# AlanPearl/multigrad

Hardware: AMD Instinct MI355X
Metric: Adam steps/sec (whole node), 1e7-param summed-loss model (higher is better)
Workload: dtype fp32; 1 GPU; global_batch=134217728, seq_len=10, parallelism=dp1, params=10000000, halos_global=134217728, optimizer=Adam (fused HIP kernel), full trajectory, graph=False, graph_steps=0, pipelined=True, placement=hashed, grad_collective=none (1 rank), sumstat_allreduce=none (1 rank), chunks=1, layout=lanes/global, bounds=none

## Files before the change

multigrad_amd/csrc/smf.hip:

```cpp
#include "common.h"
#include "twoshot.h"
#include "xgmi.h"
#include "tail_table.h"

#include <torch/extension.h>
#include <ATen/hip/HIPContext.h>
#include <cmath>
#include <vector>

namespace mg {

constexpr int kMaxBins = 32;
constexpr int kXcds = 8;
constexpr int kThreads = 256;
static_assert(kThreads == kTsThreads, "fused-exchange kernels must launch kTsThreads threads");
constexpr int kItems = 8;
constexpr int kTileHalos = kThreads * kItems;
constexpr int kTilePops = 2048;
constexpr float kLn10 = 2.302585092994046f;
constexpr float kLog2_10 = 3.321928094887362f;

struct SmfBins {
  float edge[kMaxBins + 1];
  float scale[kMaxBins];
// ... 646 lines not shown
    G[i] = G[i] + g;
    W[i] = (-g) * n + W[i];
  }
}

template <int NB, bool LOGSIG, bool REL, bool RESID, int REPL = 0>
__device__ __forceinline__ void lane_halo_ep(float x0, float x1, float ninv, float mua,
                                             const SmfBins& b,
                                             v2f (&acc)[EdgePairs<NB>::NV], int (&cnt)[NB + 1],
                                             v2f (&G)[EdgePairs<NB>::NV],
                                             v2f (&W)[EdgePairs<NB>::NV],
                                             const float4* tb = nullptr) {
  using E = EdgePairs<NB>;
  auto eval = [&](v2f n, int i, int& ca, int& cb) {
    if constexpr (REPL > 0)
      ep_eval_tab<NB, RESID, REPL>(n, tb, acc, G, W, i, ca, cb);
    else
      ep_eval<NB, REL, RESID>(n, acc, G, W, i, ca, cb);
  };
  const float mu0 = fmaf(x0, -ninv, mua);
  const float mu1 = fmaf(x1, -ninv, mua);
#pragma unroll
  for (int h = 0; h < 2; ++h) {
    const float mu = h ? mu1 : mu0;
#pragma unroll
    for (int i = 0; i < E::NP; ++i) {
      v2f e2;
      e2.x = b.edge[2 * i];
      e2.y = b.edge[2 * i + 1];
      const v2f n = e2 * ninv + mu;
      eval(n, i, cnt[2 * i], cnt[2 * i + 1]);
    }
  }
  if constexpr (E::NX) {
    v2f m2;
    m2.x = mu0;
    m2.y = mu1;
    const v2f n = (v2f)(b.edge[E::NE - 1] * ninv) + m2;
    int c2 = 0;
    eval(n, E::NP, cnt[E::NE - 1], c2);
    cnt[E::NE - 1] += c2;
  }
}

constexpr float kEmHMax = 0.5f;
constexpr float kInvSqrt2Pi = 0.39894228040143268f;

struct EmLane {
  float inv;
  float dw4;
  float a1, a3, a5;
};

__device__ __forceinline__ EmLane em_lane(float inv, float delta) {
  constexpr float ik = 1.0f / kWScale;
  EmLane L;
  L.inv = inv;
  const float dw = delta * inv;
  L.dw4 = -4.0f * dw;
  const float h = dw * ik;
  const float h2 = h * h, h4 = h2 * h2, h6 = h4 * h2;
  L.a1 = (h2 * (1.0f / 12.0f) + h4 * (3.0f / 720.0f) + h6 * (15.0f / 30240.0f)) * ik;
  L.a3 = -(h4 * (1.0f / 720.0f) + h6 * (10.0f / 30240.0f)) * (ik * ik * ik);
  L.a5 = h6 * (1.0f / 30240.0f) * (ik * ik * ik * ik * ik);
  return L;
}

constexpr float kEmH2 = 0.35f;

__device__ __forceinline__ EmLane em_lane2(float inv, float delta) {
  constexpr float ik = 1.0f / kWScale;
  EmLane L;
  L.inv = inv;
  const float dw = delta * inv;
  L.dw4 = -4.0f * dw;
  const float h = dw * ik;
  const float h2 = h * h, h4 = h2 * h2;
  L.a1 = (h2 * (1.0f / 12.0f) + h4 * (3.0f / 720.0f)) * ik;
  L.a3 = -(h4 * (1.0f / 720.0f)) * (ik * ik * ik);
  L.a5 = 0.0f;
  return L;
}

template <int NB, bool RESID, bool A7 = false, bool A5 = true>
__device__ __forceinline__ void em_halo(float nm, float inv, float dw4, float a1, float a3,
                                        float a5, const SmfBins& b,
                                        v2f (&F)[EdgePairs<NB>::NV], v2f (&Wa)[EdgePairs<NB>::NV],
                                        v2f (&E)[EdgePairs<NB>::NV], float a7 = 0.0f) {
  using EP = EdgePairs<NB>;
  constexpr int M = EP::NP / 2;
  nm = __builtin_amdgcn_fmed3f(nm, -1e6f, 1e6f);
  const float dw2 = -0.5f * dw4;
  v2f wm;
  {
    v2f e2;
    e2.x = b.edge[2 * M];
    e2.y = b.edge[2 * M + 1];
    wm = e2 * inv + nm;
  }
  auto wpair = [&](int i) { return wm + (float)(i - M) * dw2; };
  auto accum = [&](int i, v2f p, v2f w) {
    const v2f pw = p * w;
    F[i] = F[i] + p;
    if constexpr (RESID) Wa[i] = Wa[i] + pw;
    const v2f w2 = w * w;
    v2f t;
    if constexpr (A7) {
      t = w2 * a7 + a5;
      t = t * w2 + a3;
      t = t * w2 + a1;
    } else if constexpr (A5) {
      t = w2 * a5 + a3;
      t = t * w2 + a1;
    } else {
      t = w2 * a3 + a1;
    }
    E[i] = pw * t + E[i];
  };
  const v2f ws = wpair(M);
  const v2f q = -ws * ws;
  v2f p0;
  p0.x = fast_exp2(q.x);
  p0.y = fast_exp2(q.y);
  const float R = fast_exp2(__builtin_amdgcn_fmed3f(dw4 * ws.y, -126.0f, 126.0f));
  accum(M, p0, ws);
  v2f p = p0;
#pragma unroll
  for (int i = M + 1; i < EP::NP; ++i) {
    p = p * R;
    accum(i, p, wpair(i));
  }
  if constexpr (EP::NX) {
    const float pz = p.x * R;
    const float wz = fmaf((float)(EP::NP - M), dw2, wm.x);
    const float pw = pz * wz;
    F[EP::NP].x += pz;
    if constexpr (RESID) Wa[EP::NP].x += pw;
    const float w2 = wz * wz;
    const float t = A7 ? fmaf(fmaf(fmaf(w2, a7, a5), w2, a3), w2, a1)
                       : (A5 ? fmaf(fmaf(w2, a5, a3), w2, a1) : fmaf(w2, a3, a1));
    E[EP::NP].x = fmaf(pw, t, E[EP::NP].x);
  }
  if constexpr (M > 0) {
    const float Ri = fast_rcp(R);
    p = p0;
#pragma unroll
    for (int i = M - 1; i >= 0; --i) {
      p = p * Ri;
      accum(i, p, wpair(i));
    }
  }
}

template <int NB, bool RESID, bool A5 = true>
__device__ __forceinline__ void lane_halo_em(float x, const EmLane& L, float nma,
                                             const SmfBins& b, v2f (&F)[EdgePairs<NB>::NV],
                                             v2f (&Wa)[EdgePairs<NB>::NV],
                                             v2f (&E)[EdgePairs<NB>::NV]) {
  em_halo<NB, RESID, false, A5>(fmaf(x, -L.inv, nma), L.inv, L.dw4, L.a1, L.a3, L.a5, b, F, Wa, E);
  __builtin_amdgcn_sched_barrier(0);
}

template <int NB, bool RESID>
__device__ __forceinline__ void lane_halo_exact1(float x, float ninv, float mua, const SmfBins& b,
                                                 v2f (&acc)[EdgePairs<NB>::NV], int (&cnt)[NB + 1],
                                                 v2f (&G)[EdgePairs<NB>::NV],
                                                 v2f (&W)[EdgePairs<NB>::NV]) {
  const float mu = fmaf(x, -ninv, mua);
#pragma unroll
  for (int e = 0; e <= NB; ++e) {
    const float n = fmaf(b.edge[e], ninv, mu);
    float p, g;
    normal_tail_parts_w<false>(n, p, g);
    const float v = p * __builtin_copysignf(g, n);
    cnt[e] += __builtin_popcountll(__builtin_amdgcn_ballot_w64(n < 0.0f));
    const int i = e >> 1;
    if (e & 1) {
      acc[i].y += v;
      if constexpr (RESID) {
        G[i].y += g;
        W[i].y = fmaf(-g, n, W[i].y);
      }
    } else {
      acc[i].x += v;
      if constexpr (RESID) {
        G[i].x += g;
        W[i].x = fmaf(-g, n, W[i].x);
      }
    }
  }
  __builtin_amdgcn_sched_barrier(0);
}

template <int NB, class LaneT>
__device__ __forceinline__ void em_group_end(const LaneT& L, v2f (&F)[EdgePairs<NB>::NV],
                                             v2f (&Wa)[EdgePairs<NB>::NV],
                                             v2f (&E)[EdgePairs<NB>::NV],
                                             v2f (&accp)[EdgePairs<NB>::NV]) {
  using EP = EdgePairs<NB>;
  constexpr int M = EP::NP / 2;
  const float l4 = 0.25f * L.dw4 * L.dw4;
#pragma unroll
  for (int i = 0; i < EP::NV; ++i) {
    const int j = i - M;
    v2f Q;
    Q.x = (j * (j - 1) == 0) ? 1.0f : fast_exp2(-l4 * (float)(j * (j - 1)));
    Q.y = (i == EP::NP) ? Q.x : ((j * j == 0) ? 1.0f : fast_exp2(-l4 * (float)(j * j)));
    F[i] = F[i] * Q;
    Wa[i] = Wa[i] * Q;
    E[i] = E[i] * Q;
  }
  const float hh = (-0.125f / kWScale) * L.dw4;
  float T = 0.0f, fprev = 0.0f;
#pragma unroll
  for (int e = 0; e <= NB; ++e) {
    const int i = e >> 1;
    float fe, ee;
    if (i < EP::NP) {
      fe = (e & 1) ? F[i].y : F[i].x;
      ee = (e & 1) ? E[i].y : E[i].x;
    } else {
      fe = F[i].x + F[i].y;
      ee = E[i].x + E[i].y;
    }
    if (e > 0) T = fmaf(hh, fprev + fe, T);
    fprev = fe;
    const float C = kInvSqrt2Pi * (T + ee);
    if (i < EP::NP) {
      if (e & 1) accp[i].y += C;
      else accp[i].x += C;
    } else {
      accp[i].x += C;
    }
  }
}


template <int NB>
struct VjpPairs {
  v2f h[EdgePairs<NB>::NV];
  v2f d[EdgePairs<NB>::NV];
};

template <int NB>
__device__ __forceinline__ void halo_vjp_rec(float nm, float inv, float dw, const VjpPairs<NB>& W,
                                             const SmfBins& b, float& A, float& D, float& wc) {
  using EP = EdgePairs<NB>;
  constexpr int M = EP::NP / 2;
  v2f e2;
  e2.x = b.edge[2 * M];
  e2.y = b.edge[2 * M + 1];
  const v2f ws = e2 * inv + nm;
  const v2f q = -ws * ws;
  v2f p0;
  p0.x = fast_exp2(q.x);
  p0.y = fast_exp2(q.y);
  const float dw4 = -4.0f * dw;
  const float C2 = fast_exp2(dw4 * dw);
  const float C4 = C2 * C2;
  v2f Af = W.h[M] * p0, Df = W.d[M] * p0;
  v2f R;
  R.x = fast_exp2(__builtin_amdgcn_fmed3f(dw4 * ws.y, -126.0f, 126.0f));
  R.y = R.x * C2;
  v2f p = p0;
#pragma unroll
  for (int i = M + 1; i < EP::NP; ++i) {
    p = p * R;
    Af = W.h[i] * p + Af;
    Df = W.d[i] * p + Df;
    R = R * C4;
  }
  if constexpr (EP::NX) {
    const float f = p.x * R.x;
    Af.x = fmaf(W.h[EP::NP].x, f, Af.x);
    Df.x = fmaf(W.d[EP::NP].x, f, Df.x);
  }
  if constexpr (M > 0) {
    v2f Rb;
    Rb.y = fast_exp2(__builtin_amdgcn_fmed3f(-dw4 * ws.x, -126.0f, 126.0f));
    Rb.x = Rb.y * C2;
    p = p0;
#pragma unroll
    for (int i = M - 1; i >= 0; --i) {
      p = p * Rb;
      Af = W.h[i] * p + Af;
      Df = W.d[i] * p + Df;
      Rb = Rb * C4;
    }
  }
  A = Af.x + Af.y;
  D = Df.x + Df.y;
  wc = ws.x;
}

template <int NB, bool LOGSIG, int XS = 0>
#ifndef MG_VJP_REC_MINWAVES
#define MG_VJP_REC_MINWAVES 8
#endif
__global__ __launch_bounds__(kThreads, XS == 2 ? 6 : MG_VJP_REC_MINWAVES) void smf_vjp_tiles_rec_kernel(
    const float* __restrict__ x, const int32_t* __restrict__ pop,
    const float2* __restrict__ theta, const Tile* __restrict__ tiles,
    const float* __restrict__ hvec, SmfBins bins, float2* __restrict__ grad,
    float2* __restrict__ partials, TwoShotPack xs = TwoShotPack{}) {
  __shared__ __attribute__((aligned(16))) char smem[kTileHalos * (sizeof(float2) + sizeof(int16_t))];
  int tb = blockIdx.x;
  if constexpr (XS > 0) {
// ... 22 lines not shown
    block_sum_n<2>(v, reinterpret_cast<float*>(smem));
    if (tid == 0) partials[t.slot] = make_float2(v[0], v[1]);
    return;
  }
  const int n = (int)(t.h1 - t.h0);
  const int npops = t.p1 - t.p0;
  float2* __restrict__ gout = grad + t.p0;
  if (n <= 0) {
    for (int k = tid; k < npops; k += kThreads) gout[k] = make_float2(0.f, 0.f);
    return;
  }
  VjpPairs<NB> W;
#pragma unroll
  for (int i = 0; i < EP::NV; ++i) {
    const int e0 = 2 * i, e1 = 2 * i + 1;
    W.h[i].x = hvec[e0];
    W.h[i].y = e1 <= NB ? hvec[e1] : 0.0f;
    W.d[i].x = (float)(e0 - 2 * M) * W.h[i].x;
    W.d[i].y = (float)(e1 - 2 * M) * W.h[i].y;
  }
  float2* s_g = reinterpret_cast<float2*>(smem);
  int16_t* s_lp = reinterpret_cast<int16_t*>(smem + kTileHalos * sizeof(float2));
  float2* res = s_g;
  float2* s_head = reinterpret_cast<float2*>(s_lp);
  int* s_pass = reinterpret_cast<int*>(s_head + kThreads);
  static_assert(kThreads * (sizeof(float2) + sizeof(int)) <= kTileHalos * sizeof(int16_t),
                "head partials alias the id array");
  static_assert(kTileHalos == kTilePops, "result array aliases the contribution array");
  auto swz = [](int i) { return i ^ (((i >> 5) & 3) << 1); };
  {
    float xs[kItems];
    int ps[kItems];
    float2 ths[kItems];
    const float* __restrict__ xt = x + t.h0;
    const int32_t* __restrict__ pt = pop + t.h0;
#pragma unroll
    for (int r = 0; r < kItems; ++r) {
      const int i = min(r * kThreads + tid, n - 1);
      xs[r] = xt[i];
      ps[r] = pt[i];
    }
#pragma unroll
    for (int r = 0; r < kItems; ++r) ths[r] = theta[ps[r]];
    bool ok = true;
#pragma unroll
    for (int r = 0; r < kItems; ++r) ok = ok && bins.delta * inv_sigma<LOGSIG>(ths[r].y) <= 1.0f;
    constexpr float kInvW = 1.0f / kWScale;
    if (__builtin_amdgcn_ballot_w64(!ok) == 0) {
#pragma unroll
      for (int r = 0; r < kItems; ++r) {
        const float is = inv_sigma<LOGSIG>(ths[r].y);
        const float inv = is * kWScale;
        const float dw = bins.delta * inv;
        float A, D, wc;
        halo_vjp_rec<NB>(-(xs[r] + ths[r].x) * inv, inv, dw, W, bins, A, D, wc);
        const float B = fmaf(wc, A, dw * D);
        const int li = r * kThreads + tid;
        s_g[swz(li)] = make_float2(-is * A, LOGSIG ? -(kLn10 * kInvW) * B : -(is * kInvW) * B);
        s_lp[li] = (int16_t)(ps[r] - t.p0);
      }
    } else {
      float h[NB + 1];
#pragma unroll
      for (int e = 0; e <= NB; ++e) h[e] = hvec[e];
#pragma unroll
      for (int r = 0; r < kItems; ++r) {
        const float is = inv_sigma<LOGSIG>(ths[r].y);
        float A = 0.f, B = 0.f;
        halo_vjp<NB, LOGSIG>(xs[r], ths[r], is * kWScale, h, bins, A, B);
        const int li = r * kThreads + tid;
        s_g[swz(li)] = make_float2(-is * A, LOGSIG ? -(kLn10 * kInvW) * B : -(is * kInvW) * B);
        s_lp[li] = (int16_t)(ps[r] - t.p0);
      }
    }
  }
  __syncthreads();
  const int base = tid * kItems;
  const int cnt = max(0, min(kItems, n - base));
  float2 g[kItems];
  int lp[kItems];
  {
    const float4* sg4 = reinterpret_cast<const float4*>(s_g);
    const int sw = (tid >> 2) & 3;
#pragma unroll
    for (int k = 0; k < kItems / 2; ++k) {
      const float4 v = sg4[4 * tid + (k ^ sw)];
      g[2 * k] = make_float2(v.x, v.y);
      g[2 * k + 1] = make_float2(v.z, v.w);
    }
    const uint4 l4 = reinterpret_cast<const uint4*>(s_lp)[tid];
    const unsigned lw[4] = {l4.x, l4.y, l4.z, l4.w};
#pragma unroll
    for (int k = 0; k < 4; ++k) {
      lp[2 * k] = (int)(lw[k] & 0xFFFFu);
      lp[2 * k + 1] = (int)(lw[k] >> 16);
    }
  }
#pragma unroll
  for (int j = 1; j < kItems; ++j) {
    const bool in = j < cnt;
    lp[j] = in ? lp[j] : lp[j - 1];
    g[j].x = in ? g[j].x : 0.0f;
    g[j].y = in ? g[j].y : 0.0f;
  }
  const int prevlp = (cnt > 0 && base > 0) ? (int)s_lp[base - 1] : -1;
  const int nextlp = base + kItems < n ? (int)s_lp[base + kItems] : npops;
  __syncthreads();
  for (int k = tid; k < npops; k += kThreads) res[k] = make_float2(0.f, 0.f);
  __syncthreads();
  int c = lp[0];
  float2 cur = g[0];
  const bool headcont = cnt > 0 && c == prevlp;
  bool inhead = true;
  float2 hsum = make_float2(0.f, 0.f);
  if (cnt > 0) {
#pragma unroll
    for (int j = 1; j < kItems; ++j) {
      const bool brk = lp[j] != c;
      const bool hb = brk && inhead && headcont;
      if (brk && !hb) res[c] = cur;
      hsum.x = hb ? cur.x : hsum.x;
      hsum.y = hb ? cur.y : hsum.y;
      inhead = inhead && !brk;
      cur.x = brk ? g[j].x : cur.x + g[j].x;
      cur.y = brk ? g[j].y : cur.y + g[j].y;
      c = lp[j];
    }
  }
  const bool contonly = cnt > 0 && inhead && headcont;
  if (contonly) hsum = cur;
  s_head[tid] = hsum;
  s_pass[tid] = contonly && nextlp == c;
  __syncthreads();
  if (cnt > 0 && !contonly) {
    if (nextlp == c) {
      for (int k = tid + 1; k < kThreads; ++k) {
        const float2 hp = s_head[k];
        cur.x += hp.x;
        cur.y += hp.y;
        if (!s_pass[k]) break;
      }
    }
    res[c] = cur;
  }
  __syncthreads();
  for (int k = tid; k < npops; k += kThreads) gout[k] = res[k];
}

constexpr int kLanesMainMode = 3;

#ifndef MG_EM2
#define MG_EM2 1
#endif

#ifndef MG_LANES_MINWAVES
#define MG_LANES_MINWAVES 4
#endif
#ifndef MG_LANES_UNROLL
#define MG_LANES_UNROLL 2
#endif
constexpr int kLanesUnroll = MG_LANES_UNROLL;

__device__ __forceinline__ __amdgpu_buffer_rsrc_t buf_rsrc(const void* p) {
  return __builtin_amdgcn_make_buffer_rsrc(const_cast<void*>(p), (short)0, 0x7fffffff, 0x00020000);
}
__device__ __forceinline__ float buf_load_f32(__amdgpu_buffer_rsrc_t r, int voff, int soff) {
  return __builtin_bit_cast(float, __builtin_amdgcn_raw_buffer_load_b32(r, voff, soff, 0));
}
__device__ __forceinline__ int buf_load_i32(__amdgpu_buffer_rsrc_t r, int voff, int soff) {
  return (int)__builtin_amdgcn_raw_buffer_load_b32(r, voff, soff, 0);
}
__device__ __forceinline__ void buf_store_f32(__amdgpu_buffer_rsrc_t r, int voff, int soff, float v) {
  __builtin_amdgcn_raw_buffer_store_b32(__builtin_bit_cast(unsigned, v), r, voff, soff, 0);
}

struct LaneSrc {
  __amdgpu_buffer_rsrc_t r;
  int voff;
};
__device__ __forceinline__ float lane_load(const LaneSrc& xp, int j, int len) {
  return j < len ? buf_load_f32(xp.r, xp.voff, j * kWave * 4) : kLaneSentinel;
}
__device__ __forceinline__ float lane_use(float v, int j, int len) {
  return v;
}

__device__ __forceinline__ void resid_store(float* p, float v) {
  *p = v;
}

#ifdef MG_FWD_TRACE
constexpr int kTraceWaves = 16384;
__device__ unsigned long long g_fwd_trace[3 * kTraceWaves];
#endif

__device__ __forceinline__ void vmem_wait_all() { __builtin_amdgcn_s_waitcnt(0x0F70); }

template <int I>
__device__ __forceinline__ void lds_stage_chunk(const float* src, float* dst, int lane) {
  constexpr int base = (I / 4) * 1024;
  __builtin_amdgcn_global_load_lds(src + base + lane * 4, dst + base, 16, (I % 4) * 1024, 0);
}
template <int R>
__device__ __forceinline__ void lds_stage_row(const float* src, float* dst, int lane) {
  constexpr int base = (R * kWave / 1024) * 1024;
  __builtin_amdgcn_global_load_lds(src + base + lane, dst + base, 4, (R * kWave - base) * 4, 0);
}
template <int NR, int... I, int... R>
__device__ __forceinline__ void lds_stage_seq(const float* src, float* dst, int lane,
                                              std::integer_sequence<int, I...>,
                                              std::integer_sequence<int, R...>) {
  (lds_stage_chunk<I>(src, dst, lane), ...);
  (lds_stage_row<(NR / 4) * 4 + R>(src, dst, lane), ...);
}
template <int NR>
__device__ __forceinline__ void lds_stage_block(const float* src, float* dst, int lane) {
  lds_stage_seq<NR>(src, dst, lane, std::make_integer_sequence<int, NR / 4>{},
                    std::make_integer_sequence<int, NR % 4>{});
}

template <int NB>
struct LaneGroupSums {
  v2f acc[EdgePairs<NB>::NV];
  int cnt[NB + 1];
};

template <int NB>
__device__ __attribute__((noinline)) LaneGroupSums<NB> lanes_group_exact(
    const float* __restrict__ xg, int len, float x0, float x1, float ninv, float mua, float e0,
    float delta, float* __restrict__ rg) {
  using EP = EdgePairs<NB>;
  const int lane = threadIdx.x & (kWave - 1);
  SmfBins b;
#pragma unroll
  for (int e = 0; e <= NB; ++e) b.edge[e] = fmaf((float)e, delta, e0);
  LaneGroupSums<NB> o;
  v2f G[EP::NV], W[EP::NV];
#pragma unroll
  for (int i = 0; i < EP::NV; ++i) {
    o.acc[i] = (v2f)(0.0f);
    G[i] = (v2f)(0.0f);
    W[i] = (v2f)(0.0f);
  }
#pragma unroll
  for (int e = 0; e <= NB; ++e) o.cnt[e] = 0;
  const __amdgpu_buffer_rsrc_t xr = buf_rsrc(xg);
  const int voff = lane * 4;
  for (int j = 0; j < len; j += 2) {
    const float c0 = x0;
    const float c1 = j + 1 < len ? x1 : kLaneSentinel;
    x0 = buf_load_f32(xr, voff, (j + 2) * kWave * 4);
    x1 = buf_load_f32(xr, voff, (j + 3) * kWave * 4);
    lane_halo_ep<NB, true, false, true>(c0, c1, ninv, mua, b, o.acc, o.cnt, G, W);
  }
  float Gs[NB + 1], Ws[NB + 1];
#pragma unroll
  for (int i = 0; i < EP::NP; ++i) {
    Gs[2 * i] = G[i].x;
    Gs[2 * i + 1] = G[i].y;
    Ws[2 * i] = W[i].x;
    Ws[2 * i + 1] = W[i].y;
  }
  if constexpr (EP::NX) {
    Gs[NB] = G[EP::NP].x + G[EP::NP].y;
    Ws[NB] = W[EP::NP].x + W[EP::NP].y;
  }
  const __amdgpu_buffer_rsrc_t rr = buf_rsrc(rg);
#pragma unroll
  for (int e = 0; e <= NB; ++e) {
    buf_store_f32(rr, voff, e * kWave * 4, Gs[e]);
    buf_store_f32(rr, voff, (NB + 1 + e) * kWave * 4, Ws[e]);
  }
  return o;
}

template <int NB, bool LOGSIG, bool REL, bool RESID, bool UPD = false, int LMODE = 0,
          bool BND = false>
__global__ __launch_bounds__(kThreads, MG_LANES_MINWAVES) void smf_fwd_lanes_kernel(
    const float* __restrict__ xi, const int32_t* __restrict__ slot_pop,
    const int64_t* __restrict__ group_base, const int32_t* __restrict__ group_len,
    const int32_t* __restrict__ fwd_order, const float2* __restrict__ theta, int64_t g0,
    int64_t g1, SmfBins bins, float* __restrict__ slab, float* __restrict__ resid,
    const int32_t* __restrict__ wave_start, int* __restrict__ queues, int nq,
    LanesUpdate upd = LanesUpdate{}) {
  static_assert(!UPD || RESID, "the pipelined update reads the residuals it overwrites");
  static_assert(!BND || UPD, "bounds belong to the pipelined update");
  static_assert(LMODE == 0 || LMODE == 3 || LMODE == 4, "lanes mode");
  static_assert(LMODE != 3 || (RESID && !REL), "CALL: EM residual forwards");
  constexpr bool kEmOn = LMODE != 4;
  constexpr int kRepl = (!REL && !kEmOn && !RESID) ? (UPD ? 8 : 16) : 0;
  constexpr bool kEm = kEmOn && !REL;
  const float4* tb = nullptr;
  if constexpr (kRepl > 0) {
    __shared__ float4 tab[kTailTabN * (kRepl > 0 ? kRepl : 1)];
    tail_tab_fill<kRepl>(tab);
    __syncthreads();
    tb = tail_tab_lane<kRepl>(tab);
  }
  float acc[NB + 1];
  int cnt[NB + 1];
#pragma unroll
  for (int k = 0; k <= NB; ++k) {
    acc[k] = 0.0f;
    cnt[k] = 0;
  }
  using EP = EdgePairs<NB>;
  static_assert(kLanesUnroll % 2 == 0, "edge-pair path takes halos two at a time");
  v2f accp[EP::NV];
#pragma unroll
  for (int k = 0; k < EP::NV; ++k) accp[k] = (v2f)(0.0f);
  const int lane = threadIdx.x & (kWave - 1);
  const int wid = __builtin_amdgcn_readfirstlane(threadIdx.x >> 6);
  const int64_t nwaves = (int64_t)gridDim.x * (kThreads / kWave);
  const int64_t w_id = (int64_t)blockIdx.x * (kThreads / kWave) + wid;
#ifdef MG_FWD_TRACE
  const unsigned long long t_start = __builtin_amdgcn_s_memrealtime();
  int n_groups_done = 0;
#endif
  const bool dyn = queues != nullptr;
  const int qid = dyn ? (int)(blockIdx.x % nq) : 0;
  const int n_items = (int)(g1 - g0);
  const int n_q = dyn && qid < n_items ? (n_items - qid + nq - 1) / nq : 0;
  const int waves_q = dyn ? (kThreads / kWave) * (int)((gridDim.x - qid + nq - 1) / nq) : 0;
  auto draw = [&]() -> int64_t {
    int t = 0;
    if (lane == 0) {
      t = atomicAdd(queues + qid, 1);
      if (t == n_q + waves_q - 1)
        __hip_atomic_store(queues + qid, 0, __ATOMIC_RELAXED, __HIP_MEMORY_SCOPE_AGENT);
    }
    t = __builtin_amdgcn_readfirstlane(t);
    return t < n_q ? g0 + qid + (int64_t)t * nq : g1;
  };
  int64_t k = dyn ? draw() : wave_start ? (int64_t)wave_start[w_id] : g0 + w_id;
  const int64_t kstride = wave_start ? 1 : nwaves;
  if (wave_start && !dyn) g1 = wave_start[w_id + 1];
  int64_t k_next = g1;
  int64_t g = 0;
  float2 th = make_float2(0.f, 0.f);
  const int lane4 = lane * 4;
  LaneSrc xp{buf_rsrc(xi), lane4};
  auto slot_of = [&](int64_t kk) {
    return buf_load_i32(buf_rsrc(slot_pop + (int64_t)fwd_order[kk] * kWave), lane4, 0);
  };
  int len = 0;
  int c_next = 0;
  int c_cur = -1;
  float xn[kLanesUnroll];
  float ubc1 = 1.0f, ubc2 = 1.0f;
  float* utrow = nullptr;
  if constexpr (UPD) {
    const int st = upd.host_step >= 0
                       ? upd.host_step
                       : __hip_atomic_load(upd.step, __ATOMIC_RELAXED, __HIP_MEMORY_SCOPE_AGENT);
    ubc1 = 1.0f / (1.0f - powf(upd.b1, (float)(st + 1)));
    ubc2 = 1.0f / (1.0f - powf(upd.b2, (float)(st + 1)));
    if (upd.traj) utrow = upd.traj + (int64_t)(st + 1) * upd.traj_stride;
  }
  constexpr int kUR = UPD ? 2 * (NB + 1) + 4 + (BND ? 6 : 0) : 1;
  float* ubuf = nullptr;
  const float* uh = nullptr;
  if constexpr (UPD) {
    __shared__ __attribute__((aligned(16))) float ub[(kThreads / kWave) * kUR * kWave];
    __shared__ float hs[NB + 1];
    if (threadIdx.x <= NB) hs[threadIdx.x] = upd.h[threadIdx.x];
    __syncthreads();
    ubuf = ub + wid * (kUR * kWave);
    uh = hs;
  }
  auto stage_update = [&](int64_t gg, int c) {
    if constexpr (UPD) {
      constexpr int NR = 2 * (NB + 1);
      lds_stage_block<NR>(resid + gg * (NR * kWave), ubuf, lane);
      const int64_t j = c < 0 ? 0 : c - upd.unit_offset;
      const float* mp = reinterpret_cast<const float*>(upd.m + j);
      const float* vp = reinterpret_cast<const float*>(upd.v + j);
      __builtin_amdgcn_global_load_lds(mp, ubuf + NR * kWave, 4, 0, 0);
      __builtin_amdgcn_global_load_lds(mp + 1, ubuf + (NR + 1) * kWave, 4, 0, 0);
      __builtin_amdgcn_global_load_lds(vp, ubuf + (NR + 2) * kWave, 4, 0, 0);
      __builtin_amdgcn_global_load_lds(vp + 1, ubuf + (NR + 3) * kWave, 4, 0, 0);
      if constexpr (BND) {
        const float* up = reinterpret_cast<const float*>(upd.u + j);
        const float* lp = reinterpret_cast<const float*>(upd.lo + j);
        const float* hp = reinterpret_cast<const float*>(upd.hi + j);
        __builtin_amdgcn_global_load_lds(up, ubuf + (NR + 4) * kWave, 4, 0, 0);
        __builtin_amdgcn_global_load_lds(up + 1, ubuf + (NR + 5) * kWave, 4, 0, 0);
        __builtin_amdgcn_global_load_lds(lp, ubuf + (NR + 6) * kWave, 4, 0, 0);
        __builtin_amdgcn_global_load_lds(lp + 1, ubuf + (NR + 7) * kWave, 4, 0, 0);
        __builtin_amdgcn_global_load_lds(hp, ubuf + (NR + 8) * kWave, 4, 0, 0);
        __builtin_amdgcn_global_load_lds(hp + 1, ubuf + (NR + 9) * kWave, 4, 0, 0);
      }
    }
  };
  auto apply_update = [&]() {
    if constexpr (UPD) {
      constexpr int NR = 2 * (NB + 1);
      float A = 0.0f, B = 0.0f;
#pragma unroll
      for (int e = 0; e <= NB; ++e) {
        A = fmaf(uh[e], ubuf[e * kWave + lane], A);
        B = fmaf(uh[e], ubuf[(NB + 1 + e) * kWave + lane], B);
      }
      if (c_cur >= 0) {
        const float2 gr = pop_grad<LOGSIG>(th, A, B);
        const int64_t j = c_cur - upd.unit_offset;
        float2 mm = make_float2(ubuf[NR * kWave + lane], ubuf[(NR + 1) * kWave + lane]);
        float2 vv = make_float2(ubuf[(NR + 2) * kWave + lane], ubuf[(NR + 3) * kWave + lane]);
        if constexpr (BND) {
          float2 uu = make_float2(ubuf[(NR + 4) * kWave + lane], ubuf[(NR + 5) * kWave + lane]);
          const float2 lo = make_float2(ubuf[(NR + 6) * kWave + lane], ubuf[(NR + 7) * kWave + lane]);
          const float2 hi = make_float2(ubuf[(NR + 8) * kWave + lane], ubuf[(NR + 9) * kWave + lane]);
          const int8_t kx = bound_kind(lo.x, hi.x), ky = bound_kind(lo.y, hi.y);
          const float gx = gr.x * dpdu_fast(upd.legacy ? th.x : uu.x, lo.x, hi.x, kx);
          const float gy = gr.y * dpdu_fast(upd.legacy ? th.y : uu.y, lo.y, hi.y, ky);
          mm.x = (1.0f - upd.b1) * gx + upd.b1 * mm.x;
          mm.y = (1.0f - upd.b1) * gy + upd.b1 * mm.y;
          vv.x = (1.0f - upd.b2) * (gx * gx) + upd.b2 * vv.x;
          vv.y = (1.0f - upd.b2) * (gy * gy) + upd.b2 * vv.y;
          uu.x -= upd.lr * (mm.x * ubc1) * __builtin_amdgcn_rcpf(__builtin_amdgcn_sqrtf(vv.x * ubc2) + upd.eps);
          uu.y -= upd.lr * (mm.y * ubc1) * __builtin_amdgcn_rcpf(__builtin_amdgcn_sqrtf(vv.y * ubc2) + upd.eps);
          th.x = inv_transform_fast(uu.x, lo.x, hi.x, kx);
          th.y = inv_transform_fast(uu.y, lo.y, hi.y, ky);
          upd.u[j] = uu;
        } else {
          mm.x = (1.0f - upd.b1) * gr.x + upd.b1 * mm.x;
          mm.y = (1.0f - upd.b1) * gr.y + upd.b1 * mm.y;
          vv.x = (1.0f - upd.b2) * (gr.x * gr.x) + upd.b2 * vv.x;
          vv.y = (1.0f - upd.b2) * (gr.y * gr.y) + upd.b2 * vv.y;
          th.x -= upd.lr * (mm.x * ubc1) * __builtin_amdgcn_rcpf(__builtin_amdgcn_sqrtf(vv.x * ubc2) + upd.eps);
          th.y -= upd.lr * (mm.y * ubc1) * __builtin_amdgcn_rcpf(__builtin_amdgcn_sqrtf(vv.y * ubc2) + upd.eps);
        }
        upd.m[j] = mm;
        upd.v[j] = vv;
        upd.theta_w[c_cur] = th;
        if (utrow) reinterpret_cast<float2*>(utrow)[j] = th;
      }
    }
  };
  auto fetch_next_slot = [&]() {
    if (k_next < g1) c_next = slot_of(k_next);
  };
  auto load_group = [&](int64_t kk, int c, bool fetch_next = true) {
    g = fwd_order[kk];
    c_cur = c;
    stage_update(g, c);
    th = theta[c < 0 ? 0 : c];
    xp.r = buf_rsrc(xi + group_base[g]);
    len = group_len[g];
#pragma unroll
    for (int u = 0; u < kLanesUnroll; ++u) xn[u] = lane_load(xp, u, len);
    k_next = dyn ? draw() : kk + kstride;
    if (fetch_next) fetch_next_slot();
  };
  if (k < g1) {
    load_group(k, slot_of(k), !UPD);
    if constexpr (UPD) {
      vmem_wait_all();
      apply_update();
      fetch_next_slot();
    }
  }
  const int64_t k_first = k;
  while (k < g1) {
    if (!dyn && wave_start) {
      const int64_t tot = g1 - k_first;
      const int lvl = (int)((4 * (g1 - k) - 1) / tot);
      if (lvl >= 3) __builtin_amdgcn_s_setprio(3);
      else if (lvl == 2) __builtin_amdgcn_s_setprio(2);
      else if (lvl == 1) __builtin_amdgcn_s_setprio(1);
      else __builtin_amdgcn_s_setprio(0);
    }
    const int64_t gc = g;
    const float ninv = -inv_sigma<LOGSIG>(th.y) * kWScale;
    const float mua = -th.x * ninv;
    v2f Gp[EP::NV], Wp[EP::NV];
#pragma unroll
    for (int e = 0; e < EP::NV; ++e) {
      Gp[e] = (v2f)(0.0f);
      Wp[e] = (v2f)(0.0f);
    }
    bool em = false, em2 = false;
    if constexpr (kEm) {
      const float inv = -ninv;
      const float h = bins.delta * inv * (1.0f / kWScale);
      const bool bad = c_cur >= 0 && !(h <= kEmHMax);
      em = bins.delta > 0.0f && __builtin_amdgcn_ballot_w64(bad) == 0;
#if MG_EM2
      em2 = em && __builtin_amdgcn_ballot_w64(c_cur >= 0 && !(h <= kEmH2)) == 0;
#endif
    }
    if constexpr (kEm) if (em) {
      const EmLane eml = em2 ? em_lane2(-ninv, bins.delta) : em_lane(-ninv, bins.delta);
      v2f Ep[EP::NV];
#pragma unroll
      for (int e = 0; e < EP::NV; ++e) Ep[e] = (v2f)(0.0f);
      auto em_loop = [&](auto a5c) {
        for (int j = 0; j < len; j += kLanesUnroll) {
          float xc[kLanesUnroll];
#pragma unroll
          for (int u = 0; u < kLanesUnroll; ++u) {
            xc[u] = lane_use(xn[u], j + u, len);
            xn[u] = lane_load(xp, j + kLanesUnroll + u, len);
          }
#pragma unroll
          for (int u = 0; u < kLanesUnroll; ++u)
            lane_halo_em<NB, RESID, decltype(a5c)::value>(xc[u], eml, -mua, bins, Gp, Wp, Ep);
        }
      };
      if (em2) em_loop(std::false_type{});
      else em_loop(std::true_type{});
      em_group_end<NB>(eml, Gp, Wp, Ep, accp);
    }
    if constexpr (LMODE == 3) {
      if (!em) {
        const LaneGroupSums<NB> o = lanes_group_exact<NB>(
            xi + group_base[gc], len, lane_use(xn[0], 0, len), lane_use(xn[1], 1, len), ninv,
            mua, bins.edge[0], bins.delta,
            resid + gc * (2 * (NB + 1) * kWave));
#pragma unroll
        for (int i = 0; i < EP::NV; ++i) accp[i] = accp[i] + o.acc[i];
#pragma unroll
        for (int e = 0; e <= NB; ++e) cnt[e] += __builtin_amdgcn_readfirstlane(o.cnt[e]);
      }
    } else
    if (!em)
    for (int j = 0; j < len; j += kLanesUnroll) {
      float xc[kLanesUnroll];
#pragma unroll
      for (int u = 0; u < kLanesUnroll; ++u) {
        xc[u] = lane_use(xn[u], j + u, len);
        const int jn = j + kLanesUnroll + u;
        xn[u] = lane_load(xp, jn, len);
      }
      if constexpr (kEm) {
#pragma unroll
        for (int u = 0; u < kLanesUnroll; ++u)
          lane_halo_exact1<NB, RESID>(xc[u], ninv, mua, bins, accp, cnt, Gp, Wp);
      } else {
#pragma unroll
        for (int u = 0; u < kLanesUnroll; u += 2)
          lane_halo_ep<NB, LOGSIG, REL, RESID, kRepl>(xc[u], xc[u + 1], ninv, mua, bins, accp,
                                                      cnt, Gp, Wp, tb);
      }
    }
    const int64_t kn = k_next;
#ifdef MG_FWD_TRACE
    ++n_groups_done;
#endif
    if constexpr (!UPD)
      if (kn < g1) load_group(kn, c_next);
    if (RESID && (LMODE != 3 || em)) {
      const __amdgpu_buffer_rsrc_t rr = buf_rsrc(resid + gc * (2 * (NB + 1) * kWave));
      float G[NB + 1], W[NB + 1];
#pragma unroll
      for (int i = 0; i < EP::NP; ++i) {
        G[2 * i] = Gp[i].x;
        G[2 * i + 1] = Gp[i].y;
        W[2 * i] = Wp[i].x;
        W[2 * i + 1] = Wp[i].y;
      }
      if constexpr (EP::NX) {
        G[NB] = Gp[EP::NP].x + Gp[EP::NP].y;
        W[NB] = Wp[EP::NP].x + Wp[EP::NP].y;
      }
#pragma unroll
      for (int e = 0; e <= NB; ++e) {
        buf_store_f32(rr, lane4, e * kWave * 4, G[e]);
        buf_store_f32(rr, lane4, (NB + 1 + e) * kWave * 4, W[e]);
      }
    }
    k = kn;
    if constexpr (UPD) {
      if (k < g1) {
        load_group(k, c_next, false);
        vmem_wait_all();
        apply_update();
        fetch_next_slot();
      }
    }
  }
#pragma unroll
  for (int i = 0; i < EP::NP; ++i) {
    acc[2 * i] = accp[i].x;
    acc[2 * i + 1] = accp[i].y;
  }
  if constexpr (EP::NX) acc[NB] = accp[EP::NP].x + accp[EP::NP].y;
#ifdef MG_FWD_TRACE
  if (lane == 0 && w_id < kTraceWaves) {
    g_fwd_trace[3 * w_id] = t_start;
    g_fwd_trace[3 * w_id + 1] = __builtin_amdgcn_s_memrealtime();
    g_fwd_trace[3 * w_id + 2] = (unsigned long long)n_groups_done;
  }
#endif
  const bool counter = lane == 0;
#pragma unroll
  for (int k = 0; k < NB; ++k)
    acc[k] = (acc[k + 1] - acc[k]) + (counter ? (float)(cnt[k + 1] - cnt[k]) : 0.0f);
  __shared__ float scratch[NB * (kThreads / kWave)];
  float(&bin)[NB] = *reinterpret_cast<float(*)[NB]>(acc);
  block_sum_n<NB>(bin, scratch);
  if (threadIdx.x == 0) {
#pragma unroll
    for (int k = 0; k < NB; ++k) slab[(int64_t)blockIdx.x * NB + k] = acc[k];
  }
}

struct VjpAdam {
  float2* theta;
  float2* m;
  float2* v;
  float2* traj;
  int64_t traj_stride;
  int64_t unit_offset;
  const int* step;
  int host_step;
  float lr, b1, b2, eps;
};

__device__ __forceinline__ void adam_pair(const VjpAdam& o, float bc1, float bc2, float2 g,
                                          float2& u, float2& m, float2& v) {
  m.x = (1.0f - o.b1) * g.x + o.b1 * m.x;
  m.y = (1.0f - o.b1) * g.y + o.b1 * m.y;
  v.x = (1.0f - o.b2) * (g.x * g.x) + o.b2 * v.x;
  v.y = (1.0f - o.b2) * (g.y * g.y) + o.b2 * v.y;
  u.x = u.x - o.lr * (m.x / bc1) / (sqrtf(v.x / bc2) + o.eps);
  u.y = u.y - o.lr * (m.y / bc1) / (sqrtf(v.y / bc2) + o.eps);
}

__global__ void smf_advance_step_kernel(int* step) { step[0] += 1; }

template <int NB, bool LOGSIG, bool ADAM = false>
__global__ __launch_bounds__(kThreads) void smf_vjp_lanes_kernel(
    const int32_t* __restrict__ slot_pop, const int32_t* __restrict__ slot_part,
    const float2* theta, const float* __restrict__ hvec,
    const float* __restrict__ resid, int64_t s0, int64_t s1,
    float2* __restrict__ grad, float2* __restrict__ partials, VjpAdam adam = VjpAdam{}) {
  float bc1 = 1.0f, bc2 = 1.0f;
  float2* trow = nullptr;
  if constexpr (ADAM) {
    const int st = adam.host_step >= 0
                       ? adam.host_step
                       : __hip_atomic_load(adam.step, __ATOMIC_RELAXED, __HIP_MEMORY_SCOPE_AGENT);
    bc1 = 1.0f - powf(adam.b1, (float)(st + 1));
    bc2 = 1.0f - powf(adam.b2, (float)(st + 1));
    if (adam.traj)
      trow = reinterpret_cast<float2*>(reinterpret_cast<float*>(adam.traj) +
                                       (int64_t)(st + 1) * adam.traj_stride);
  }
  constexpr int R = 2 * (NB + 1);
  const int lane = threadIdx.x & (kWave - 1);
  const int64_t g0 = s0 / kWave, g1 = s1 / kWave;
  const int xcd = blockIdx.x % kXcds;
  const int64_t nbx = gridDim.x / kXcds;
  const int64_t ngx = (g1 - g0 + kXcds - 1) / kXcds;
  const int64_t ga = g0 + xcd * ngx, gb = min(g1, ga + ngx);
  const int64_t nw = nbx * (kThreads / kWave);
  int64_t g = ga + (int64_t)(blockIdx.x / kXcds) * (kThreads / kWave) + (threadIdx.x >> 6);
  float r[R];
  int c = -1, part = -1;
  if (g < gb) {
#pragma unroll
    for (int e = 0; e < R; ++e) r[e] = resid[(g * R + e) * kWave + lane];
    c = slot_pop[g * kWave + lane];
    part = slot_part[g * kWave + lane];
  }
  while (g < gb) {
    float A = 0.0f, B = 0.0f;
#pragma unroll
    for (int e = 0; e <= NB; ++e) {
      A = fmaf(hvec[e], r[e], A);
      B = fmaf(hvec[e], r[NB + 1 + e], B);
    }
    const int cc = c, pp = part;
    const int64_t gn = g + nw;
    if (gn < gb) {
#pragma unroll
      for (int e = 0; e < R; ++e) r[e] = resid[(gn * R + e) * kWave + lane];
      c = slot_pop[gn * kWave + lane];
      part = slot_part[gn * kWave + lane];
    }
    if (cc >= 0) {
      if (pp >= 0) {
        partials[pp] = make_float2(A, B);
      } else if constexpr (ADAM) {
        float2 u = theta[cc];
        const float2 gr = pop_grad<LOGSIG>(u, A, B);
        const int64_t j = cc - adam.unit_offset;
        float2 mm = adam.m[j], vv = adam.v[j];
        adam_pair(adam, bc1, bc2, gr, u, mm, vv);
        adam.m[j] = mm;
        adam.v[j] = vv;
        adam.theta[cc] = u;
        if (trow) trow[j] = u;
      } else {
        grad[cc] = pop_grad<LOGSIG>(theta[cc], A, B);
      }
    }
    g = gn;
  }
}

template <int NB, bool LOGSIG>
__global__ __launch_bounds__(kThreads) void smf_vjp_lanes_rc_kernel(
    const float* __restrict__ xi, const int32_t* __restrict__ slot_idx,
    const int32_t* __restrict__ slot_part, const int64_t* __restrict__ group_base,
    const int32_t* __restrict__ group_len, const float2* __restrict__ theta,
    const float* __restrict__ hvec, SmfBins bins, int64_t g0, int64_t g1,
    float2* __restrict__ grad, float2* __restrict__ partials) {
  float h[NB + 1];
#pragma unroll
  for (int e = 0; e <= NB; ++e) h[e] = hvec[e];
  const int lane = threadIdx.x & (kWave - 1);
  const int64_t nw = (int64_t)gridDim.x * (kThreads / kWave);
  for (int64_t g = g0 + (int64_t)blockIdx.x * (kThreads / kWave) + (threadIdx.x >> 6); g < g1;
       g += nw) {
    const int64_t s = g * kWave + lane;
    const int c = slot_idx[s];
    const float2 th = theta[c < 0 ? 0 : c];
    const float inv = inv_sigma<LOGSIG>(th.y) * kWScale;
    const int len = group_len[g];
    const float* xp = xi + group_base[g] + lane;
    float A = 0.0f, B = 0.0f;
    int j = 0;
    for (; j + 2 <= len; j += 2) {
      const float x0 = xp[(int64_t)j * kWave];
      const float x1 = xp[(int64_t)(j + 1) * kWave];
      halo_vjp<NB, LOGSIG>(x0, th, inv, h, bins, A, B);
      halo_vjp<NB, LOGSIG>(x1, th, inv, h, bins, A, B);
    }
    if (j < len) halo_vjp<NB, LOGSIG>(xp[(int64_t)j * kWave], th, inv, h, bins, A, B);
    if (c >= 0) {
      const int part = slot_part[s];
      if (part >= 0) partials[part] = make_float2(A, B);
      else grad[c] = pop_grad<LOGSIG>(th, A, B);
    }
  }
}

__global__ __launch_bounds__(kThreads) void smf_lanes_pack_kernel(
    const float* __restrict__ xs, const int64_t* __restrict__ slot_src,
    const int32_t* __restrict__ slot_len, const int64_t* __restrict__ group_base,
    const int32_t* __restrict__ group_len, int64_t ngroups, float* __restrict__ xi) {
  const int lane = threadIdx.x & (kWave - 1);
  const int64_t g = (int64_t)blockIdx.x * (kThreads / kWave) + (threadIdx.x >> 6);
  if (g >= ngroups) return;
  const int64_t s = g * kWave + lane;
  const int64_t src = slot_src[s];
  const int len = slot_len[s];
  const int glen = group_len[g];
  float* dst = xi + group_base[g] + lane;
  for (int j = 0; j < glen; ++j) dst[(int64_t)j * kWave] = j < len ? xs[src + j] : kLaneSentinel;
}

static int padded_bins(int nb) {
  const int sizes[] = {1, 2, 4, 8, 10, 16, 32};
  for (int s : sizes)
    if (nb <= s) return s;
  TORCH_CHECK(false, "at most ", kMaxBins, " bins supported, got ", nb);
  return 0;
}

static SmfBins make_bins(const std::vector<double>& edges, const std::vector<double>& scale, int nbp) {
  const int nb = (int)scale.size();
  TORCH_CHECK((int)edges.size() == nb + 1, "need nb+1 edges");
  SmfBins b;
  for (int e = 0; e <= kMaxBins; ++e) b.edge[e] = (float)edges[std::min(e, nb)];
  for (int k = 0; k < kMaxBins; ++k) b.scale[k] = k < nb ? (float)scale[k] : 0.0f;
  const double d = (edges[nb] - edges[0]) / nb;
  bool uni = nb == nbp && d > 0;
  for (int e = 0; e <= nb && uni; ++e)
    uni = std::fabs(edges[e] - (edges[0] + e * d)) <= 1e-6 * std::max(1.0, std::fabs(edges[e]));
  b.delta = uni ? (float)d : 0.0f;
  return b;
}

#define MG_DISPATCH_NB(NBP, ...)                             \
  switch (NBP) {                                             \
    case 1: { constexpr int NB = 1; __VA_ARGS__; break; }    \
    case 2: { constexpr int NB = 2; __VA_ARGS__; break; }    \
    case 4: { constexpr int NB = 4; __VA_ARGS__; break; }    \
    case 8: { constexpr int NB = 8; __VA_ARGS__; break; }    \
    case 10: { constexpr int NB = 10; __VA_ARGS__; break; }  \
    case 16: { constexpr int NB = 16; __VA_ARGS__; break; }  \
    default: { constexpr int NB = 32; __VA_ARGS__; break; }  \
  }

static void check_dev(const torch::Tensor& t, const char* name, at::ScalarType st) {
  TORCH_CHECK(t.is_cuda(), name, " must be a device tensor");
  TORCH_CHECK(t.is_contiguous(), name, " must be contiguous");
  TORCH_CHECK(t.scalar_type() == st, name, " has wrong dtype");
}

int smf_padded_bins(int64_t nb) { return padded_bins((int)nb); }

template <typename F>
static void with_bool(bool v, F&& f) {
  if (v) f(std::true_type{});
  else f(std::false_type{});
}

int64_t smf_fwd_max_blocks(int64_t nb, bool log_sigma, bool has_pop, bool rel_tail) {
  const int nbp = padded_bins((int)nb);
  int dev = 0;
  hipGetDevice(&dev);
  hipDeviceProp_t prop;
  hipGetDeviceProperties(&prop, dev);
  int occ = 0;
  MG_DISPATCH_NB(nbp, {
    with_bool(log_sigma, [&](auto LS) { with_bool(has_pop, [&](auto HP) { with_bool(rel_tail, [&](auto RT) {
      const void* f = (const void*)smf_fwd_kernel<NB, decltype(LS)::value, decltype(HP)::value, decltype(RT)::value>;
      (void)hipOccupancyMaxActiveBlocksPerMultiprocessor(&occ, f, kThreads, 0);
    }); }); });
  });
  return (int64_t)std::max(1, occ) * prop.multiProcessorCount;
}

void smf_forward(torch::Tensor x, c10::optional<torch::Tensor> pop, torch::Tensor theta,
                 std::vector<double> edges, std::vector<double> scale, bool log_sigma,
                 int64_t begin, int64_t end, torch::Tensor slab, int64_t nblocks, bool rel_tail,
                 std::string exchange) {
  check_dev(x, "x", at::kFloat);
  check_dev(theta, "theta", at::kFloat);
  check_dev(slab, "slab", at::kFloat);
  const int nbp = padded_bins((int)scale.size());
  TORCH_CHECK(begin >= 0 && end <= x.numel() && begin <= end, "bad halo range");
  TORCH_CHECK(slab.numel() >= nblocks * nbp, "slab too small");
  TORCH_CHECK(nblocks >= 1 && nblocks <= 65535, "bad block count");
  const bool has_pop = pop.has_value() && pop->defined();
  if (has_pop) {
    check_dev(*pop, "pop", at::kInt);
// ... 1316 lines not shown
```

Measured before the change: 2202 steps/s.

## Interleave residual blocks per lane for 128-bit vector stores and loads

Changes the per-group residual layout from one row per element across lanes to lane-interleaved quads, so each lane writes four consecutive floats. The forward lanes kernel, the pipelined update and the backward/Adam pass now use b128/b64 buffer stores and float4/float2 loads in place of scalar ones. This cuts the number of memory instructions for residual traffic. The cost is that the LDS-staged update path reads 16-byte strides per lane, which may cause bank conflicts. Every producer and consumer of the residual buffer must agree on the new layout.

```diff
diff --git a/multigrad_amd/csrc/smf.hip b/multigrad_amd/csrc/smf.hip
--- a/multigrad_amd/csrc/smf.hip
+++ b/multigrad_amd/csrc/smf.hip
@@ -1183,9 +1183,58 @@
   return v;
 }
 
-__device__ __forceinline__ void resid_store(float* p, float v) {
-  *p = v;
-}
+template <int NB>
+struct ResidBlock {
+  static constexpr int R = 2 * (NB + 1);
+  static constexpr int NQ = R / 4;
+  static constexpr bool PAIR = R % 4 == 2;
+  static_assert(R % 2 == 0 && NQ * 4 + (PAIR ? 2 : 0) == R, "quads plus at most one pair");
+  static constexpr int kFloats = R * kWave;
+  static constexpr int quad(int q) { return q * 4 * kWave; }
+  static constexpr int pair() { return NQ * 4 * kWave; }
+  static __device__ __forceinline__ float pick(const float (&G)[NB + 1], const float (&W)[NB + 1],
+                                               int r) {
+    return r <= NB ? G[r] : W[r - (NB + 1)];
+  }
+  static __device__ __forceinline__ void store(float* blk, int lane4,
+                                               const float (&G)[NB + 1], const float (&W)[NB + 1]) {
+    typedef unsigned u4 __attribute__((ext_vector_type(4)));
+    typedef unsigned u2 __attribute__((ext_vector_type(2)));
+    auto bits = [](float v) { return __builtin_bit_cast(unsigned, v); };
+#pragma unroll
+    for (int q = 0; q < NQ; ++q) {
+      u4 v;
+      v.x = bits(pick(G, W, 4 * q));
+      v.y = bits(pick(G, W, 4 * q + 1));
+      v.z = bits(pick(G, W, 4 * q + 2));
+      v.w = bits(pick(G, W, 4 * q + 3));
+      __builtin_amdgcn_raw_buffer_store_b128(v, buf_rsrc(blk + quad(q / 4 * 4)),
+                                             lane4 * 4 + quad(q % 4) * 4, 0, 0);
+    }
+    if constexpr (PAIR) {
+      u2 v;
+      v.x = bits(pick(G, W, R - 2));
+      v.y = bits(pick(G, W, R - 1));
+      __builtin_amdgcn_raw_buffer_store_b64(v, buf_rsrc(blk + quad(NQ / 4 * 4)),
+                                            lane4 * 2 + quad(NQ % 4) * 4, 0, 0);
+    }
+  }
+  static __device__ __forceinline__ void load(const float* blk, int lane4, float (&r)[R]) {
+#pragma unroll
+    for (int q = 0; q < NQ; ++q) {
+      const float4 v = *reinterpret_cast<const float4*>(blk + quad(q) + lane4);
+      r[4 * q] = v.x;
+      r[4 * q + 1] = v.y;
+      r[4 * q + 2] = v.z;
+      r[4 * q + 3] = v.w;
+    }
+    if constexpr (PAIR) {
+      const float2 v = *reinterpret_cast<const float2*>(blk + pair() + lane4 / 2);
+      r[R - 2] = v.x;
+      r[R - 1] = v.y;
+    }
+  }
+};
 
 #ifdef MG_FWD_TRACE
 constexpr int kTraceWaves = 16384;
@@ -1263,12 +1312,7 @@
     Gs[NB] = G[EP::NP].x + G[EP::NP].y;
     Ws[NB] = W[EP::NP].x + W[EP::NP].y;
   }
-  const __amdgpu_buffer_rsrc_t rr = buf_rsrc(rg);
-#pragma unroll
-  for (int e = 0; e <= NB; ++e) {
-    buf_store_f32(rr, voff, e * kWave * 4, Gs[e]);
-    buf_store_f32(rr, voff, (NB + 1 + e) * kWave * 4, Ws[e]);
-  }
+  ResidBlock<NB>::store(rg, voff, Gs, Ws);
   return o;
 }
 
@@ -1337,6 +1381,11 @@
   int64_t g = 0;
   float2 th = make_float2(0.f, 0.f);
   const int lane4 = lane * 4;
+  auto lane4_here = [&]() {
+    int v = lane4;
+    asm volatile("" : "+v"(v));
+    return v;
+  };
   LaneSrc xp{buf_rsrc(xi), lane4};
   auto slot_of = [&](int64_t kk) {
     return buf_load_i32(buf_rsrc(slot_pop + (int64_t)fwd_order[kk] * kWave), lane4, 0);
@@ -1369,7 +1418,7 @@
   auto stage_update = [&](int64_t gg, int c) {
     if constexpr (UPD) {
       constexpr int NR = 2 * (NB + 1);
-      lds_stage_block<NR>(resid + gg * (NR * kWave), ubuf, lane);
+      lds_stage_block<NR>(resid + gg * ResidBlock<NB>::kFloats, ubuf, lane);
       const int64_t j = c < 0 ? 0 : c - upd.unit_offset;
       const float* mp = reinterpret_cast<const float*>(upd.m + j);
       const float* vp = reinterpret_cast<const float*>(upd.v + j);
@@ -1394,10 +1443,12 @@
     if constexpr (UPD) {
       constexpr int NR = 2 * (NB + 1);
       float A = 0.0f, B = 0.0f;
+      float r[NR];
+      ResidBlock<NB>::load(ubuf, lane4_here(), r);
 #pragma unroll
       for (int e = 0; e <= NB; ++e) {
-        A = fmaf(uh[e], ubuf[e * kWave + lane], A);
-        B = fmaf(uh[e], ubuf[(NB + 1 + e) * kWave + lane], B);
+        A = fmaf(uh[e], r[e], A);
+        B = fmaf(uh[e], r[NB + 1 + e], B);
       }
       if (c_cur >= 0) {
         const float2 gr = pop_grad<LOGSIG>(th, A, B);
@@ -1514,7 +1565,7 @@
         const LaneGroupSums<NB> o = lanes_group_exact<NB>(
             xi + group_base[gc], len, lane_use(xn[0], 0, len), lane_use(xn[1], 1, len), ninv,
             mua, bins.edge[0], bins.delta,
-            resid + gc * (2 * (NB + 1) * kWave));
+            resid + gc * ResidBlock<NB>::kFloats);
 #pragma unroll
         for (int i = 0; i < EP::NV; ++i) accp[i] = accp[i] + o.acc[i];
 #pragma unroll
@@ -1548,7 +1599,6 @@
     if constexpr (!UPD)
       if (kn < g1) load_group(kn, c_next);
     if (RESID && (LMODE != 3 || em)) {
-      const __amdgpu_buffer_rsrc_t rr = buf_rsrc(resid + gc * (2 * (NB + 1) * kWave));
       float G[NB + 1], W[NB + 1];
 #pragma unroll
       for (int i = 0; i < EP::NP; ++i) {
@@ -1561,11 +1611,7 @@
         G[NB] = Gp[EP::NP].x + Gp[EP::NP].y;
         W[NB] = Wp[EP::NP].x + Wp[EP::NP].y;
       }
-#pragma unroll
-      for (int e = 0; e <= NB; ++e) {
-        buf_store_f32(rr, lane4, e * kWave * 4, G[e]);
-        buf_store_f32(rr, lane4, (NB + 1 + e) * kWave * 4, W[e]);
-      }
+      ResidBlock<NB>::store(resid + gc * ResidBlock<NB>::kFloats, lane4_here(), G, W);
     }
     k = kn;
     if constexpr (UPD) {
@@ -1657,8 +1703,7 @@
   float r[R];
   int c = -1, part = -1;
   if (g < gb) {
-#pragma unroll
-    for (int e = 0; e < R; ++e) r[e] = resid[(g * R + e) * kWave + lane];
+    ResidBlock<NB>::load(resid + g * ResidBlock<NB>::kFloats, lane * 4, r);
     c = slot_pop[g * kWave + lane];
     part = slot_part[g * kWave + lane];
   }
@@ -1672,8 +1717,7 @@
     const int cc = c, pp = part;
     const int64_t gn = g + nw;
     if (gn < gb) {
-#pragma unroll
-      for (int e = 0; e < R; ++e) r[e] = resid[(gn * R + e) * kWave + lane];
+      ResidBlock<NB>::load(resid + gn * ResidBlock<NB>::kFloats, lane * 4, r);
       c = slot_pop[gn * kWave + lane];
       part = slot_part[gn * kWave + lane];
     }
```

After: 2202 steps/s, median of 3. No clear change (+0.0%).

## Accumulate per-bin power moments in EM path and reconstruct polynomial terms once per group

Applied to the files above, without the earlier changes.

For the em2 case with residuals and 8 or 10 bins, the per-halo edge loop now accumulates raw moments (sum p, p*w, p*w^2, p*w^3) about a single centre point. The shifted polynomial terms are rebuilt per bin once at the end of the group via a binomial expansion. This drops the per-halo per-edge polynomial evaluation and the per-edge w shift in favour of a few vector FMAs. The cost is an extra accumulator array, which raises register pressure, and some risk of cancellation error in the end-of-group expansion.

```diff
diff --git a/multigrad_amd/csrc/smf.hip b/multigrad_amd/csrc/smf.hip
--- a/multigrad_amd/csrc/smf.hip
+++ b/multigrad_amd/csrc/smf.hip
@@ -822,6 +822,93 @@
   }
 }
 
+template <int NB>
+__device__ __forceinline__ void em_halo_moments(float nm, float inv, float dw4, const SmfBins& b,
+                                                v2f (&S0)[EdgePairs<NB>::NV],
+                                                v2f (&S1)[EdgePairs<NB>::NV],
+                                                v2f (&S2)[EdgePairs<NB>::NV],
+                                                v2f (&S3)[EdgePairs<NB>::NV]) {
+  using EP = EdgePairs<NB>;
+  constexpr int M = EP::NP / 2;
+  nm = __builtin_amdgcn_fmed3f(nm, -1e6f, 1e6f);
+  v2f wm;
+  {
+    v2f e2;
+    e2.x = b.edge[2 * M];
+    e2.y = b.edge[2 * M + 1];
+    wm = e2 * inv + nm;
+  }
+  const v2f u2 = wm * wm;
+  const v2f u3 = u2 * wm;
+  auto accum = [&](int i, v2f p) {
+    S0[i] = S0[i] + p;
+    S1[i] = p * wm + S1[i];
+    S2[i] = p * u2 + S2[i];
+    S3[i] = p * u3 + S3[i];
+  };
+  v2f p0;
+  p0.x = fast_exp2(-u2.x);
+  p0.y = fast_exp2(-u2.y);
+  const float R = fast_exp2(__builtin_amdgcn_fmed3f(dw4 * wm.y, -126.0f, 126.0f));
+  accum(M, p0);
+  v2f p = p0;
+#pragma unroll
+  for (int i = M + 1; i < EP::NP; ++i) {
+    p = p * R;
+    accum(i, p);
+  }
+  if constexpr (EP::NX) {
+    const float pz = p.x * R;
+    S0[EP::NP].x += pz;
+    S1[EP::NP].x = fmaf(pz, wm.x, S1[EP::NP].x);
+    S2[EP::NP].x = fmaf(pz, u2.x, S2[EP::NP].x);
+    S3[EP::NP].x = fmaf(pz, u3.x, S3[EP::NP].x);
+  }
+  if constexpr (M > 0) {
+    const float Ri = fast_rcp(R);
+    p = p0;
+#pragma unroll
+    for (int i = M - 1; i >= 0; --i) {
+      p = p * Ri;
+      accum(i, p);
+    }
+  }
+}
+
+template <int NB>
+__device__ __forceinline__ void em_moments_end(float dw4, float a1, float a3,
+                                               const v2f (&S0)[EdgePairs<NB>::NV],
+                                               v2f (&S1)[EdgePairs<NB>::NV],
+                                               const v2f (&S2)[EdgePairs<NB>::NV],
+                                               v2f (&S3)[EdgePairs<NB>::NV]) {
+  using EP = EdgePairs<NB>;
+  constexpr int M = EP::NP / 2;
+  const float dw2 = -0.5f * dw4;
+#pragma unroll
+  for (int i = 0; i < EP::NV; ++i) {
+    v2f c = S3[i];
+    if (i != M) {
+      const float s = (float)(i - M) * dw2;
+      c = S0[i] * s + 3.0f * S1[i];
+      c = c * s + 3.0f * S2[i];
+      c = c * s + S3[i];
+      S1[i] = S0[i] * s + S1[i];
+    }
+    S3[i] = S1[i] * a1 + c * a3;
+  }
+}
+
+template <int NB>
+__device__ __forceinline__ void lane_halo_em_moments(float x, const EmLane& L, float nma,
+                                                     const SmfBins& b,
+                                                     v2f (&S0)[EdgePairs<NB>::NV],
+                                                     v2f (&S1)[EdgePairs<NB>::NV],
+                                                     v2f (&S2)[EdgePairs<NB>::NV],
+                                                     v2f (&S3)[EdgePairs<NB>::NV]) {
+  em_halo_moments<NB>(fmaf(x, -L.inv, nma), L.inv, L.dw4, b, S0, S1, S2, S3);
+  __builtin_amdgcn_sched_barrier(0);
+}
+
 template <int NB, bool RESID, bool A5 = true>
 __device__ __forceinline__ void lane_halo_em(float x, const EmLane& L, float nma,
                                              const SmfBins& b, v2f (&F)[EdgePairs<NB>::NV],
@@ -1150,6 +1237,11 @@
 #ifndef MG_EM2
 #define MG_EM2 1
 #endif
+#ifndef MG_EM_MOMENTS
+#define MG_EM_MOMENTS 1
+#endif
+template <int NB, bool RESID>
+constexpr bool kEmMomentsFor = MG_EM_MOMENTS != 0 && RESID && (NB == 8 || NB == 10);
 
 #ifndef MG_LANES_MINWAVES
 #define MG_LANES_MINWAVES 4
@@ -1288,6 +1380,7 @@
   constexpr bool kEmOn = LMODE != 4;
   constexpr int kRepl = (!REL && !kEmOn && !RESID) ? (UPD ? 8 : 16) : 0;
   constexpr bool kEm = kEmOn && !REL;
+  constexpr bool kEmMoments = kEm && kEmMomentsFor<NB, RESID>;
   const float4* tb = nullptr;
   if constexpr (kRepl > 0) {
     __shared__ float4 tab[kTailTabN * (kRepl > 0 ? kRepl : 1)];
@@ -1492,7 +1585,7 @@
       v2f Ep[EP::NV];
 #pragma unroll
       for (int e = 0; e < EP::NV; ++e) Ep[e] = (v2f)(0.0f);
-      auto em_loop = [&](auto a5c) {
+      auto halo_loop = [&](auto&& halo) {
         for (int j = 0; j < len; j += kLanesUnroll) {
           float xc[kLanesUnroll];
 #pragma unroll
@@ -1501,12 +1594,29 @@
             xn[u] = lane_load(xp, j + kLanesUnroll + u, len);
           }
 #pragma unroll
-          for (int u = 0; u < kLanesUnroll; ++u)
-            lane_halo_em<NB, RESID, decltype(a5c)::value>(xc[u], eml, -mua, bins, Gp, Wp, Ep);
+          for (int u = 0; u < kLanesUnroll; ++u) halo(xc[u]);
         }
       };
-      if (em2) em_loop(std::false_type{});
-      else em_loop(std::true_type{});
+      auto em_loop = [&](auto a5c) {
+        halo_loop([&](float x) {
+          lane_halo_em<NB, RESID, decltype(a5c)::value>(x, eml, -mua, bins, Gp, Wp, Ep);
+        });
+      };
+      if (em2) {
+        if constexpr (kEmMoments) {
+          v2f S2[EP::NV];
+#pragma unroll
+          for (int e = 0; e < EP::NV; ++e) S2[e] = (v2f)(0.0f);
+          halo_loop([&](float x) {
+            lane_halo_em_moments<NB>(x, eml, -mua, bins, Gp, Wp, S2, Ep);
+          });
+          em_moments_end<NB>(eml.dw4, eml.a1, eml.a3, Gp, Wp, S2, Ep);
+        } else {
+          em_loop(std::false_type{});
+        }
+      } else {
+        em_loop(std::true_type{});
+      }
       em_group_end<NB>(eml, Gp, Wp, Ep, accp);
     }
     if constexpr (LMODE == 3) {
```

Measured after the change: 2314 steps/s before, 2316 steps/s after, median of 3. About the same (+0.1%).
